# adamjorr/kbbq

Measured on AMD Instinct MI355X. Metric: recalibrated Gbases/sec, higher is better.
Workload: dtype u64

## Files before the change

### kbbq_amd/csrc/bucket.h

```cpp
#pragma once
#include <hip/hip_runtime.h>
#include <stdint.h>

#include "device_common.h"

namespace kbbq {

constexpr int SUB_BITS = 12;
constexpr int NB2_BITS = 9;
constexpr int SUB_BLOCKS = 1 << SUB_BITS;
constexpr int NB2 = 1 << NB2_BITS;
constexpr int L1_SHIFT = SUB_BITS + NB2_BITS;
constexpr int MAX_NB1 = 512;
constexpr int N_XCD = 8;
constexpr int CNT_STRIDE = 32;
constexpr int BK_THREADS = 512;
constexpr int EMIT_GRID = 512;

struct BucketDev {
    unsigned long long *l1;
    uint32_t *l1_cnt;
    uint32_t *l2;
    uint32_t *l2_cnt;
    uint32_t *tickets;
    unsigned long long *direct;
    uint32_t cap1, cap2;
    int nb1;
    int n_src;
    int cnt_stride;
    uint32_t n_sub;
};

__device__ __forceinline__ int xcc_id() {
    unsigned x;
    asm volatile("s_getreg_b32 %0, hwreg(HW_REG_XCC_ID, 0, 4)" : "=s"(x));
    return (int)(x & (N_XCD - 1));
}

__device__ __forceinline__ uint32_t block_scan512(uint32_t v, uint32_t *wave_tot, uint32_t *total) {
    const int lane = threadIdx.x & 63, w = threadIdx.x >> 6;
    uint32_t inc = v;
#pragma unroll
    for (int o = 1; o < 64; o <<= 1) { const uint32_t y = __shfl_up(inc, o); if (lane >= o) inc += y; }
    if (lane == 63) wave_tot[w] = inc;
    __syncthreads();
    uint32_t before = 0, all = 0;
#pragma unroll
    for (int i = 0; i < 8; ++i) { const uint32_t t = wave_tot[i]; before += i < w ? t : 0; all += t; }
    *total = all;
    return before + inc - v;
}

template <int NW, int CH, bool BY_BASE, int RPW, bool PRIV, bool DENSE = true>
__global__ void __launch_bounds__(BK_THREADS) k_emit_marked(ReadsDev R, KParams K, FiltDev F, BucketDev B, const uint64_t *mask,
                                                             uint64_t mask_words, const uint64_t *kofs,
                                                             unsigned long long *inserted) {
    using S = Stage<NW>;
    constexpr int SLOTS = RPW * CH;
    extern __shared__ unsigned long long sorted[];
    __shared__ uint32_t stage[8][DENSE ? RPW : 1][2 * S::WORDS];
    __shared__ uint32_t hist[MAX_NB1], ofs_l[MAX_NB1], gbase_l[MAX_NB1], fill_l[MAX_NB1], wave_tot[8];
    const int lane = threadIdx.x & 63;
    const int w = __builtin_amdgcn_readfirstlane(threadIdx.x >> 6);
    uint32_t *L32 = stage[w][0];
    const int k = K.k;
    const int src = PRIV ? (int)blockIdx.x : xcc_id();
    const uint64_t reads_per_tile = 8 * RPW;
    const uint64_t n_tiles = (R.n_reads + reads_per_tile - 1) / reads_per_tile;
    unsigned long long mine = 0, direct = 0;
    hist[threadIdx.x] = 0;
    if (PRIV) fill_l[threadIdx.x] = (int)threadIdx.x < B.nb1 ? B.l1_cnt[(size_t)src * B.nb1 + threadIdx.x] : 0u;
    __syncthreads();
    uint64_t off[RPW], kb[RPW], word[RPW];
    uint32_t len[RPW];
    auto fetch_tile = [&](uint64_t tile) {
        const uint64_t r0 = (tile * 8 + w) * RPW;
#pragma unroll
        for (int rr = 0; rr < RPW; ++rr) {
            off[rr] = 0; kb[rr] = 0; word[rr] = 0; len[rr] = 0;
            if (r0 + rr < R.n_reads) {
                read_span(R, r0 + rr, off[rr], len[rr]);
                kb[rr] = BY_BASE ? off[rr] : kmer_base(kofs, r0 + rr, R.read_len, k);
                word[rr] = stage_fetch<NW>(R, nullptr, mask, kb[rr], mask_words - 1, off[rr], lane);
            }
        }
    };
    if (blockIdx.x < n_tiles) fetch_tile(blockIdx.x);
    for (uint64_t tile = blockIdx.x; tile < n_tiles; tile += gridDim.x) {
        unsigned long long rec[SLOTS];
        int rk[SLOTS];
#pragma unroll
        for (int s = 0; s < SLOTS; ++s) { rec[s] = 0; rk[s] = -1; }
        if (DENSE) {
            unsigned long long *wlist = sorted + (size_t)w * SLOTS * 64;
            int n_dense = 0;
            __builtin_amdgcn_wave_barrier();
            if (lane < S::WORDS) {
#pragma unroll
                for (int rr = 0; rr < RPW; ++rr) stage_store(stage[w][rr], lane, word[rr]);
            }
            __builtin_amdgcn_wave_barrier();
#pragma unroll
            for (int rr = 0; rr < RPW; ++rr) {
                const int nk = (int)len[rr] - k + 1;
                if (nk > 0) {
                    const uint32_t *L32 = stage[w][rr];
                    const int o31 = (int)(off[rr] & 31), o63 = (int)(off[rr] & 63), x63 = (int)(kb[rr] & 63);
#pragma unroll
                    for (int c = 0; c < CH; ++c) {
                        if (c * 64 < nk) {
                            const int s = c * 64 + lane;
                            const bool marked = lds_bit(L32 + 2 * S::X, x63 + s) != 0;
                            const bool valid = (lds_window32(L32 + 2 * S::M, o63 + s) & K.nmask_bits) == 0;
                            const bool take = s < nk && marked && (BY_BASE || valid);
                            const unsigned long long bal = __ballot(take);
                            if (take) wlist[n_dense + __popcll(bal & ((1ULL << lane) - 1))] = lds_window64(L32 + 2 * S::B, 2 * (o31 + s));
                            n_dense += (int)__popcll(bal);
                            if (!BY_BASE && R.hint_sampled) or_bits64(R.hint_sampled, off[rr] + (uint64_t)c * 64, bal, lane);
                            mine += __popcll(bal);
                        }
                    }
                }
            }
            __builtin_amdgcn_wave_barrier();
#pragma unroll
            for (int i = 0; i < SLOTS; ++i) {
                if (i * 64 < n_dense && i * 64 + lane < n_dense) {
                    const uint64_t key = canon_key(wlist[i * 64 + lane], K);
                    const uint32_t blk = block_of(F, key);
                    rec[i] = ((unsigned long long)blk << 16) | pattern_of(F, key);
                    rk[i] = (int)atomicAdd(&hist[blk >> L1_SHIFT], 1u);
                }
            }
        } else {
#pragma unroll
        for (int rr = 0; rr < RPW; ++rr) {
            const int nk = (int)len[rr] - k + 1;
            if (nk > 0) {
                __builtin_amdgcn_wave_barrier();
                if (lane < S::WORDS) stage_store(L32, lane, word[rr]);
                __builtin_amdgcn_wave_barrier();
                const int o31 = (int)(off[rr] & 31), o63 = (int)(off[rr] & 63), x63 = (int)(kb[rr] & 63);
#pragma unroll
                for (int c = 0; c < CH; ++c) {
                    if (c * 64 < nk) {
                        const int s = c * 64 + lane;
                        const bool marked = lds_bit(L32 + 2 * S::X, x63 + s) != 0;
                        const bool valid = (lds_window32(L32 + 2 * S::M, o63 + s) & K.nmask_bits) == 0;
                        const bool take = s < nk && marked && (BY_BASE || valid);
                        const uint64_t key = canon_key(lds_window64(L32 + 2 * S::B, 2 * (o31 + s)), K);
                        const uint32_t blk = block_of(F, key);
                        rec[rr * CH + c] = ((unsigned long long)blk << 16) | pattern_of(F, key);
                        if (take) rk[rr * CH + c] = (int)atomicAdd(&hist[blk >> L1_SHIFT], 1u);
                        const unsigned long long bal = __ballot(take);
                        if (!BY_BASE && R.hint_sampled) or_bits64(R.hint_sampled, off[rr] + (uint64_t)c * 64, bal, lane);
                        mine += __popcll(bal);
                    }
                }
            }
        }
        }
        if (tile + gridDim.x < n_tiles) fetch_tile(tile + gridDim.x);
        __syncthreads();
        const uint32_t cnt = hist[threadIdx.x];
        hist[threadIdx.x] = 0;
        uint32_t g = 0;
        if (PRIV) {
            g = fill_l[threadIdx.x];
            fill_l[threadIdx.x] = g + cnt;
        } else if (cnt) {
            g = atomicAdd(&B.l1_cnt[((size_t)src * B.nb1 + threadIdx.x) * CNT_STRIDE], cnt);
        }
        uint32_t total;
        const uint32_t ex = block_scan512(cnt, wave_tot, &total);
        ofs_l[threadIdx.x] = ex;
        gbase_l[threadIdx.x] = g;
        __syncthreads();
#pragma unroll
        for (int s = 0; s < SLOTS; ++s)
            if (rk[s] >= 0) sorted[ofs_l[(uint32_t)(rec[s] >> (16 + L1_SHIFT))] + (uint32_t)rk[s]] = rec[s];
        __syncthreads();
        for (uint32_t i = threadIdx.x; i < total; i += BK_THREADS) {
            const unsigned long long v = sorted[i];
            const uint32_t b = (uint32_t)(v >> (16 + L1_SHIFT));
            const uint32_t pos = gbase_l[b] + (i - ofs_l[b]);
            if (pos < B.cap1) {
                B.l1[((size_t)src * B.nb1 + b) * B.cap1 + pos] = v;
            } else {
                bloom_put(F, (uint32_t)(v >> 16), (uint32_t)(v & 0xFFFFu));
                ++direct;
            }
        }
        if (DENSE) __syncthreads();
    }
    if (PRIV && (int)threadIdx.x < B.nb1) B.l1_cnt[(size_t)src * B.nb1 + threadIdx.x] = fill_l[threadIdx.x];
    if (inserted && lane == 0 && mine) atomicAdd(inserted, mine);
    if (direct) atomicAdd(B.direct, direct);
}

constexpr int SPLIT_PER_THREAD = 12;
constexpr int SPLIT_TILE = BK_THREADS * SPLIT_PER_THREAD;

__global__ void __launch_bounds__(BK_THREADS) k_split(FiltDev F, BucketDev B, uint32_t chunks_per_region) {
    __shared__ uint32_t hist[NB2], ofs_l[NB2], gbase_l[NB2], wave_tot[8], unit_l;
    __shared__ uint32_t sorted[SPLIT_TILE];
    __shared__ uint16_t sorted_b[SPLIT_TILE];
    const int home = xcc_id();
    unsigned long long direct = 0;
    hist[threadIdx.x] = 0;
    for (int qi = 0; qi < N_XCD; ++qi) {
        const int q = (home + qi) & (N_XCD - 1);
        const uint32_t n_buckets = B.nb1 > q ? (uint32_t)(B.nb1 - q + N_XCD - 1) / N_XCD : 0;
        const uint32_t n_units = n_buckets * (uint32_t)B.n_src * chunks_per_region;
        for (;;) {
            __syncthreads();
            if (threadIdx.x == 0) unit_l = atomicAdd(&B.tickets[q * CNT_STRIDE], 1u);
            __syncthreads();
            const uint32_t unit = unit_l;
            if (unit >= n_units) break;
            const uint32_t chunk = unit % chunks_per_region, rest = unit / chunks_per_region;
            const int x = (int)(rest % (uint32_t)B.n_src), b1 = q + (int)(rest / (uint32_t)B.n_src) * N_XCD;
            const size_t region = (size_t)x * B.nb1 + b1;
            const uint32_t n = min(B.l1_cnt[region * B.cnt_stride], B.cap1);
            const uint32_t first = chunk * (uint32_t)SPLIT_TILE;
            if (first >= n) continue;
            const uint32_t m = min((uint32_t)SPLIT_TILE, n - first);
            const unsigned long long *src = B.l1 + region * B.cap1 + first;
            uint32_t rec[SPLIT_PER_THREAD];
            int rk[SPLIT_PER_THREAD];
#pragma unroll
            for (int j = 0; j < SPLIT_PER_THREAD; ++j) {
                const uint32_t i = j * BK_THREADS + threadIdx.x;
                rk[j] = -1;
                rec[j] = 0;
                if (i < m) {
                    const unsigned long long v = src[i];
                    rec[j] = (uint32_t)v;
                    rk[j] = (int)atomicAdd(&hist[(uint32_t)(v >> (16 + SUB_BITS)) & (NB2 - 1)], 1u);
                    rk[j] |= (int)(((uint32_t)(v >> (16 + SUB_BITS)) & (NB2 - 1)) << 16);
                }
            }
            __syncthreads();
            const uint32_t cnt = hist[threadIdx.x];
            hist[threadIdx.x] = 0;
            uint32_t g = 0;
            if (cnt) g = atomicAdd(&B.l2_cnt[(size_t)b1 * NB2 + threadIdx.x], cnt);
            uint32_t total;
            const uint32_t ex = block_scan512(cnt, wave_tot, &total);
            ofs_l[threadIdx.x] = ex;
            gbase_l[threadIdx.x] = g;
            __syncthreads();
#pragma unroll
            for (int j = 0; j < SPLIT_PER_THREAD; ++j)
                if (rk[j] >= 0) {
                    const uint32_t b2 = (uint32_t)rk[j] >> 16, at = ofs_l[b2] + ((uint32_t)rk[j] & 0xFFFFu);
                    sorted[at] = rec[j] & 0x0FFFFFFFu;
                    sorted_b[at] = (uint16_t)b2;
                }
            __syncthreads();
            for (uint32_t i = threadIdx.x; i < total; i += BK_THREADS) {
                const uint32_t v = sorted[i], b2 = sorted_b[i];
                const uint32_t pos = gbase_l[b2] + (i - ofs_l[b2]);
                const size_t sub = (size_t)b1 * NB2 + b2;
                if (pos < B.cap2) {
                    B.l2[sub * B.cap2 + pos] = v;
                } else {
                    bloom_put(F, (uint32_t)(sub << SUB_BITS) | (v >> 16), v & 0xFFFFu);
                    ++direct;
                }
            }
        }
    }
    if (direct) atomicAdd(B.direct, direct);
}

constexpr int APPLY_THREADS = 1024;

__global__ void __launch_bounds__(APPLY_THREADS) k_apply(FiltDev F, BucketDev B) {
// ... 46 lines not shown
```

### kbbq_amd/csrc/engine.hip

```cpp
#include <hip/hip_runtime.h>

#include <algorithm>
#include <climits>
#include <cstdarg>
#include <cstdio>
#include <cstdlib>
#include <cstring>
#include <map>
#include <mutex>
#include <string>
#include <thread>
#include <vector>

#include "../../include/kbbq_engine.h"
#include "abi_internal.h"
#include "correct.h"
#include "correct_wave.h"
#include "device_common.h"
#include "host_model.h"

using namespace kbbq;

static thread_local char g_err[512] = "";
int kbbq_fail(int code, const char *fmt, ...) {
    va_list ap;
    va_start(ap, fmt);
    vsnprintf(g_err, sizeof g_err, fmt, ap);
    va_end(ap);
    return code;
}
#define fail kbbq_fail
#define HIP_TRY(expr)                                                                                  \
    do {                                                                                               \
        hipError_t _e = (expr);                                                                        \
        if (_e != hipSuccess)                                                                          \
            return fail(_e == hipErrorOutOfMemory ? KBBQ_ENOMEM : KBBQ_EIO, "%s: %s (%s:%d)", #expr,   \
                        hipGetErrorString(_e), __FILE__, __LINE__);                                    \
    } while (0)

#include "kernels.h"
#include "bucket.h"
#include "long_reads.h"
#include "fixed_compare.h"


struct FilterHost {
    FilterSpec spec;
    uint64_t *d_table = nullptr;
    uint64_t *d_patterns = nullptr;
    unsigned long long *d_inserted = nullptr;
    uint64_t table_bytes() const { return spec.n_blocks * kEngineBlockBytes; }
    FiltDev dev() const {
        FiltDev f;
        f.table = reinterpret_cast<ulonglong2 *>(d_table);
        f.patterns = reinterpret_cast<const ulonglong2 *>(d_patterns);
        f.n_blocks = spec.n_blocks;
        const ModMagic mm = make_mod_magic(spec.n_blocks);
        f.mod_magic = mm.m64;
        f.mod_m32 = mm.m32;
        f.salt0 = spec.salt[0];
        f.salt1 = spec.salt[1];
        return f;
    }
};

struct ProfileSlot {
    std::string name;
    uint64_t launches = 0;
    double ms = 0;
};
struct PendingEvent {
    int slot;
    hipEvent_t a, b;
};

constexpr int kNoOverride = INT_MIN;
struct Options {
    bool no_overlap = false;
    bool no_fastpath = false;
    bool lane_walk = false;
    bool no_pass4_pipeline = false;
    int pass2_side = 2;
    bool tally_general = false;
    bool infer_subset = true;
    bool debug_bucket = false;
    int bucket = -1;
    uint64_t bucket_records = 0;
    uint64_t pass4_piece = 0;
    int scan_blocks = -1;
    int walk_blocks = -1;
    int infer_blocks = 0;
    int subset_edge = kNoOverride;
    int subset_pmask = kNoOverride;
};


enum Scratch {
    S_KMER_PREFIX,
    S_HOST_OUT,
    S_HOST_FLAGS,
    S_DRAW0, S_DRAW1,
    S_TAKE1,
    S_READ_INDEX0, S_READ_INDEX1,
    S_TMASK, S_DIRTY, S_LIST, S_ERR, S_PATCH,
    S_OFFCASE_LIST,
    S_WALK_WORDS,
    S_SIDE1,
    S_COUNT = S_SIDE1 + (S_SIDE1 - S_TMASK),
    S_TAKE0 = S_ERR + (S_SIDE1 - S_TMASK),
};
constexpr int per_side(Scratch name, int side) { return name + side * (S_SIDE1 - S_TMASK); }

struct SideCounters { unsigned long long list_len, queries; };
struct Counters {
    SideCounters side0;
    unsigned long long kmer_total;
    unsigned long long infer_fetched;
    SideCounters side1;
    unsigned long long offcase_len[2];
    SideCounters *side(int s) { return s ? &side1 : &side0; }
};
struct Tickets {
    unsigned int infer, scan[2], walk[2], unused[11];
};
struct Totals {
    unsigned long long walk_reads, walk_queries;
    unsigned long long digest, unused;
};
static_assert(sizeof(Counters) == 64 && offsetof(Counters, kmer_total) == 16 && offsetof(Counters, side1) == 32 && offsetof(Counters, offcase_len) == 48, "d_counters");
static_assert(sizeof(Tickets) == 64 && offsetof(Tickets, scan) == 4 && offsetof(Tickets, walk) == 12, "d_tickets");
static_assert(sizeof(Totals) == 32 && offsetof(Totals, digest) == 16, "d_totals");

struct Pass3 {
    int side;
    hipStream_t stream;
    int stream_no;
    unsigned long long *cnt;
    unsigned int *scan_ticket, *wave_ticket;
    bool shared;
};

struct kbbq_engine {
    kbbq_params p;
    Options opt;
    KParams K;
    hipStream_t stream = nullptr;
    hipStream_t stream2 = nullptr;
    hipEvent_t ev_main = nullptr, ev_side[2] = {nullptr, nullptr};
    hipEvent_t ev_draw = nullptr, ev_ins[2] = {nullptr, nullptr};
    bool ins_pending[2] = {false, false};
    int draw_turn = 0;
    bool side_busy[2] = {false, false};
    Totals *d_totals = nullptr;
    int side_turn = 0;
    uint32_t *d_qpresent = nullptr;
    uint32_t qpresent[8] = {};
    bool qpresent_known = false;
    uint8_t *d_dq_qslot = nullptr;
    int dq_slots = 0;
    uint32_t *d_rg_present[2] = {nullptr, nullptr};
    FilterHost filt[2];
    Xoshiro256 seed_state;
    uint64_t draw_threshold = 0;
    bool draw_always = false;
    bool thresholds_set = false;
    std::vector<int32_t> thresholds;
    unsigned long long *d_hist = nullptr;
// ... 520 lines not shown
        if (!b.est_pending && b.h_inserted) {
            HIP_TRY(hipMemcpyAsync(b.h_inserted, e->filt[1].d_inserted, 8, hipMemcpyDeviceToHost, e->stream));
            HIP_TRY(hipEventRecord(b.ev_est, e->stream));
            b.est_pending = true;
            b.est_bases = b.bases_since[1] + b.cur_bases;
            b.est_prev = b.inserted_at_flush[1];
            if (!b.est_known) {
                HIP_TRY(hipEventSynchronize(b.ev_est));
                bucket_poll_estimate(e);
                b.est_known = true;
            }
        }
    }
    if (e->opt.debug_bucket) fprintf(stderr, "[bucket] flush %d of filter %d: estimate %.3g records over %llu bases (%.4f per base), barrier %d\n",
                       (int)b.flushes[w], w, b.pending_est[w], (unsigned long long)b.bases_since[w], w ? b.frac_trusted : 0.0, (int)barrier);
    b.bases_since[w] = 0;
    b.pending[w] = false;
    b.pending_est[w] = 0;
    b.flushes[w] += 1;
    return KBBQ_OK;
}

int bucket_flush_all(kbbq_engine *e) {
    for (int w = 0; w < 2; ++w) {
        int rc = bucket_flush(e, w);
        if (rc) return rc;
    }
    return KBBQ_OK;
}

int settle(kbbq_engine *e) {
    int rc = bucket_flush_all(e);
    return rc ? rc : sync_engine(e);
}

int bucket_reserve(kbbq_engine *e, int w, double est, uint64_t bases) {
    kbbq_engine::Buckets &b = e->bk;
    int rc = bucket_flush(e, 1 - w);
    if (rc) return rc;
    b.cur_bases = bases;
    if (b.pending[w] && b.pending_est[w] + est > 0.93 * (double)b.capacity) {
        if ((rc = bucket_flush(e, w, false))) return rc;
        if (w == 1) est = (est - 4096.0) / std::max(1e-9, b.frac_used) * b.frac_trusted + 4096.0;
    }
    b.cur_bases = 0;
    b.pending[w] = true;
    b.pending_est[w] += est;
    b.bases_since[w] += bases;
    return KBBQ_OK;
}

}


extern "C" {

const char *kbbq_last_error(void) { return g_err; }

int kbbq_engine_create(const kbbq_params *params, kbbq_engine **out) {
    if (!params || !out) return fail(KBBQ_EINVAL, "null argument");
    if (params->k < 1 || params->k > KBBQ_MAX_KMER) return fail(KBBQ_ERANGE, "k must be <= %d and > 0", KBBQ_MAX_KMER);
    if (params->n_rg < 1 || params->n_rg > 65535) return fail(KBBQ_EINVAL, "n_rg must be in 1..65535");
    if (params->max_read_len < 1 || params->max_read_len > KBBQ_MAX_READ_LEN)
        return fail(KBBQ_ERANGE, "max_read_len must be in 1..%d", KBBQ_MAX_READ_LEN);
    int ndev = 0;
    if (hipGetDeviceCount(&ndev) != hipSuccess || ndev == 0) return fail(KBBQ_ENODEV, "no HIP device visible");
    if (params->device < 0 || params->device >= ndev) return fail(KBBQ_ENODEV, "device %d of %d", params->device, ndev);
    DeviceGuard create_guard(params->device);
    HIP_TRY(create_guard.err);
    kbbq_engine *e = new kbbq_engine;
    e->p = *params;
    {
        Options &o = e->opt;
        auto env_set = [](const char *name) { const char *v = getenv(name); return v && *v; };
        auto env_int = [](const char *name, int dflt) { const char *v = getenv(name); return v && *v ? atoi(v) : dflt; };
        const int fl = params->flags;
        o.no_overlap = (fl & KBBQ_F_NO_OVERLAP) || env_set("KBBQ_NO_OVERLAP");
        o.no_fastpath = (fl & KBBQ_F_NO_FASTPATH) || env_set("KBBQ_NO_FASTPATH");
        o.lane_walk = (fl & KBBQ_F_LANE_WALK) || (getenv("KBBQ_CORRECT") && !strcmp(getenv("KBBQ_CORRECT"), "lane"));
        o.no_pass4_pipeline = (fl & KBBQ_F_NO_PASS4_PIPELINE) || env_set("KBBQ_NO_PASS4_PIPELINE");
        o.pass2_side = (fl & KBBQ_F_PASS2_INORDER) ? 0 : env_int("KBBQ_PASS2_SIDE", o.pass2_side);
        o.tally_general = env_set("KBBQ_TALLY_GENERAL");
        o.infer_subset = env_int("KBBQ_INFER_SUBSET", 1) != 0;
        o.debug_bucket = env_set("KBBQ_DEBUG_BUCKET");
        o.bucket = (fl & KBBQ_F_BUCKET_ON) ? 1 : (fl & KBBQ_F_BUCKET_OFF) ? 0 : env_set("KBBQ_BUCKET") ? (env_int("KBBQ_BUCKET", 0) != 0 ? 1 : 0) : -1;
        o.bucket_records = env_u64("KBBQ_BUCKET_RECORDS", 0);
        o.pass4_piece = env_u64("KBBQ_PASS4_PIECE", 0);
        o.scan_blocks = env_int("KBBQ_SCAN_BLOCKS", o.scan_blocks);
        o.walk_blocks = env_int("KBBQ_WALK_BLOCKS", o.walk_blocks);
        o.infer_blocks = env_int("KBBQ_INFER_BLOCKS", o.infer_blocks);
        o.subset_edge = env_int("KBBQ_SUBSET_EDGE", o.subset_edge);
        o.subset_pmask = env_int("KBBQ_SUBSET_PMASK", o.subset_pmask);
    }
    e->K.k = params->k;
    e->K.shift = 2u * (unsigned)(params->k - 1);
    e->K.mask = params->k < 32 ? ((1ULL << (2 * params->k)) - 1) : ~0ULL;
    e->K.nmask_bits = params->k < 32 ? ((1u << params->k) - 1) : 0xFFFFFFFFu;
    const double fprs[2] = {params->fpr_sampled, params->fpr_trusted};
    for (int w = 0; w < 2; ++w) {
        if (!make_filter_spec(params->approx_kmers, fprs[w], params->bloom_seed, e->filt[w].spec)) {
            delete e;
            return fail(KBBQ_EINVAL, "Error: Invalid bloom filter parameters. Adjust parameters and try again.");
        }
    }
    hipError_t he = hipStreamCreateWithFlags(&e->stream, hipStreamNonBlocking);
    if (he == hipSuccess) he = hipStreamCreateWithFlags(&e->stream2, hipStreamNonBlocking);
    if (he == hipSuccess) he = hipStreamCreateWithFlags(&e->copy, hipStreamNonBlocking);
    for (hipEvent_t *ev : engine_events(e))
        if (he == hipSuccess) he = hipEventCreateWithFlags(ev, hipEventDisableTiming);
    if (he == hipSuccess) he = hipHostMalloc((void **)&e->bk.h_inserted, 64, hipHostMallocDefault);
    if (he != hipSuccess) { kbbq_engine_destroy(e); return fail(KBBQ_EIO, "hipStreamCreate: %s", hipGetErrorString(he)); }
#define CREATE_TRY(expr)                                                                           \
    do {                                                                                           \
        hipError_t _e = (expr);                                                                    \
        if (_e != hipSuccess) {                                                                    \
            int code = _e == hipErrorOutOfMemory ? KBBQ_ENOMEM : KBBQ_EIO;                         \
            fail(code, "%s: %s", #expr, hipGetErrorString(_e));                                    \
            kbbq_engine_destroy(e);                                                                \
            return code;                                                                           \
        }                                                                                          \
    } while (0)
    CREATE_TRY(hipMalloc(&e->d_counters, sizeof(Counters)));
    CREATE_TRY(hipMemset(e->d_counters, 0, sizeof(Counters)));
    CREATE_TRY(hipMalloc(&e->d_tickets, sizeof(Tickets)));
    CREATE_TRY(hipMemset(e->d_tickets, 0, sizeof(Tickets)));
    CREATE_TRY(hipMalloc(&e->d_totals, sizeof(Totals)));
    CREATE_TRY(hipMemset(e->d_totals, 0, sizeof(Totals)));
    CREATE_TRY(hipMalloc(&e->d_dq_qslot, KBBQ_NQ));
    CREATE_TRY(hipMalloc(&e->d_qpresent, 32));
    for (int i = 0; i < 2; ++i) CREATE_TRY(hipMalloc(&e->d_rg_present[i], (((size_t)params->n_rg + 31) / 32) * 4 + 4));
    for (int w = 0; w < 2; ++w) {
        FilterHost &f = e->filt[w];
        CREATE_TRY(hipMalloc(&f.d_table, f.table_bytes()));
        CREATE_TRY(hipMalloc(&f.d_patterns, kNumPatterns * kEngineBlockBytes));
        CREATE_TRY(hipMalloc(&f.d_inserted, 8));
        std::vector<uint64_t> packed(kNumPatterns * 2);
        for (uint64_t i = 0; i < kNumPatterns; ++i) {
            if (!squeeze_block(&f.spec.patterns[i * 8], &packed[i * 2])) {
                kbbq_engine_destroy(e);
                return fail(KBBQ_ESTATE, "pattern %llu uses a bit outside the 128 the generator can reach", (unsigned long long)i);
            }
        }
        CREATE_TRY(hipMemcpy(f.d_patterns, packed.data(), kNumPatterns * kEngineBlockBytes, hipMemcpyHostToDevice));
    }
    e->hist_cycle_words = (uint64_t)params->n_rg * kNQ * 2 * params->max_read_len * 2;
    e->hist_dinuc_words = (uint64_t)params->n_rg * kNQ * 16 * 2;
    CREATE_TRY(hipMalloc(&e->d_hist, (e->hist_cycle_words + e->hist_dinuc_words) * 8));
    CREATE_TRY(hipMalloc(&e->d_dq_base, (size_t)params->n_rg * kNQ * 2));
    CREATE_TRY(hipMalloc(&e->d_dq_cycle, (size_t)params->n_rg * kNQ * 2 * params->max_read_len));
    CREATE_TRY(hipMalloc(&e->d_dq_dinuc, (size_t)params->n_rg * kNQ * 16));
    CREATE_TRY(hipMemcpyToSymbol(HIP_SYMBOL(c_jump), xoshiro_jump_table(), 64 * 4 * 8));
    e->seed_state.seed32(params->seed);
    e->draw_threshold = bernoulli_threshold(params->alpha, &e->draw_always);
    int rc = kbbq_engine_reset(e);
    if (rc) { kbbq_engine_destroy(e); return rc; }
    CREATE_TRY(hipDeviceSynchronize());
    *out = e;
    return KBBQ_OK;
}

void kbbq_engine_destroy(kbbq_engine *e) {
    if (!e) return;
    DeviceGuard destroy_guard(e->p.device);
    if (e->stream) { hipStreamSynchronize(e->stream); }
    if (e->stream2) hipStreamSynchronize(e->stream2);
    if (e->copy) hipStreamSynchronize(e->copy);
// ... 4 lines not shown
    if (e->copy) hipStreamDestroy(e->copy);
    if (e->bk.h_inserted) hipHostFree(e->bk.h_inserted);
    for (int w = 0; w < 2; ++w) {
        hipFree(e->filt[w].d_table);
        hipFree(e->filt[w].d_patterns);
        hipFree(e->filt[w].d_inserted);
    }
    hipFree(e->d_hist);
    hipFree(e->d_dq_base);
    hipFree(e->d_dq_cycle);
    hipFree(e->d_dq_dinuc);
    hipFree(e->d_counters);
    hipFree(e->d_tickets);
    hipFree(e->d_totals);
    hipFree(e->d_dq_qslot);
    hipFree(e->d_qpresent);
    hipFree(e->d_rg_present[0]);
    hipFree(e->d_rg_present[1]);
    hipFree(e->d_qcum);
    hipFree(e->d_errthr);
    hipFree(e->bk.l1); hipFree(e->bk.l2); hipFree(e->bk.l1_cnt); hipFree(e->bk.l2_cnt); hipFree(e->bk.tickets); hipFree(e->bk.direct);
    for (int i = 0; i < S_COUNT; ++i) hipFree(e->scratch[i]);
    if (e->stream2) { hipStreamSynchronize(e->stream2); hipStreamDestroy(e->stream2); }
    if (e->stream) hipStreamDestroy(e->stream);
    delete e;
}

int kbbq_engine_reset(kbbq_engine *e) {
    ENGINE_DEVICE(e);
    int rc0 = sync_engine(e);
    if (rc0) return rc0;
    for (int w = 0; w < 2; ++w) {
        HIP_TRY(hipMemsetAsync(e->filt[w].d_table, 0, e->filt[w].table_bytes(), e->stream));
        HIP_TRY(hipMemsetAsync(e->filt[w].d_inserted, 0, 8, e->stream));
    }
    HIP_TRY(hipMemsetAsync(e->d_hist, 0, (e->hist_cycle_words + e->hist_dinuc_words) * 8, e->stream));
    HIP_TRY(hipMemsetAsync(e->d_counters, 0, sizeof(Counters), e->stream));
    HIP_TRY(hipMemsetAsync(e->d_totals, 0, offsetof(Totals, digest), e->stream));
    HIP_TRY(hipMemsetAsync(e->d_qpresent, 0, 32, e->stream));
    memset(e->qpresent, 0, sizeof e->qpresent);
    e->qpresent_known = false;
    if (e->bk.allocated) {
        HIP_TRY(hipMemsetAsync(e->bk.l1_cnt, 0, kL1CntBytes, e->stream));
        HIP_TRY(hipMemsetAsync(e->bk.l2_cnt, 0, kL2CntBytes, e->stream));
        HIP_TRY(hipMemsetAsync(e->bk.direct, 0, 8, e->stream));
    }
    e->bk.est_pending = false;
    e->bk.est_known = false;
    e->bk.frac_trusted = 0.75;
    e->bk.stream[0] = e->bk.stream[1] = nullptr;
    for (int w = 0; w < 2; ++w) { e->bk.pending[w] = false; e->bk.pending_est[w] = 0; e->bk.bases_since[w] = 0; e->bk.inserted_at_flush[w] = 0; e->bk.flushes[w] = 0; }
    e->thresholds_set = false;
    e->dq_set = false;
    memset(e->stats, 0, sizeof e->stats);
    return sync_engine(e);
}

int kbbq_engine_sync(kbbq_engine *e) {
    ENGINE_DEVICE(e);
    return settle(e);
}

void *kbbq_engine_stream(kbbq_engine *e) { return e ? (void *)e->stream : nullptr; }

int kbbq_engine_dims(kbbq_engine *e, uint64_t *n_rg, uint64_t *n_cycle) {
    if (!e) return fail(KBBQ_EINVAL, "null engine");
    if (n_rg) *n_rg = (uint64_t)e->p.n_rg;
    if (n_cycle) *n_cycle = (uint64_t)e->p.max_read_len;
    return KBBQ_OK;
}

int kbbq_engine_tune(kbbq_engine *e, const char *name, uint64_t value) {
    if (!e || !name) return fail(KBBQ_EINVAL, "null argument");
    if (!strcmp(name, "bucket_records")) {
        if (e->bk.allocated) return fail(KBBQ_ESTATE, "the record buffers are allocated already");
        e->opt.bucket_records = value;
    } else if (!strcmp(name, "pass4_piece")) {
        e->opt.pass4_piece = value;
    } else if (!strcmp(name, "scan_blocks") || !strcmp(name, "walk_blocks") || !strcmp(name, "infer_blocks")) {
        if (value > 17) return fail(KBBQ_EINVAL, "%s: 0 (as many as fit) to 16 workgroups per CU, 17 = default", name);
        (name[0] == 's' ? e->opt.scan_blocks : name[0] == 'w' ? e->opt.walk_blocks : e->opt.infer_blocks) = value == 17 ? (name[0] == 'i' ? 0 : -1) : (int)value;
    } else if (!strcmp(name, "infer_subset")) {
        e->opt.infer_subset = value != 0;
    } else if (!strcmp(name, "pass2_side") || !strcmp(name, "no_overlap")) {
        ENGINE_DEVICE(e);
        int rc = settle(e);
        if (rc) return rc;
        if (name[0] == 'p' && value > 2) return fail(KBBQ_EINVAL, "pass2_side: 0, 1 or 2");
        if (name[0] == 'p') e->opt.pass2_side = (int)value; else e->opt.no_overlap = value != 0;
        e->bk.stream[0] = e->bk.stream[1] = nullptr;
    } else {
        return fail(KBBQ_EINVAL, "unknown knob '%s'", name);
    }
    return KBBQ_OK;
}

int kbbq_filter_info_get(kbbq_engine *e, int which, kbbq_filter_info *out) {
    ENGINE_DEVICE(e);
    if (!out || which < 0 || which > 1) return fail(KBBQ_EINVAL, "bad argument");
    int rc = settle(e);
    if (rc) return rc;
    const FilterSpec &s = e->filt[which].spec;
    memset(out, 0, sizeof *out);
    out->bits = s.bits;
    out->bits_unblocked = s.bits_unblocked;
    out->n_blocks = s.n_blocks;
    out->table_bytes = e->filt[which].table_bytes();
    out->random_seed = s.random_seed;
    out->n_hash = s.n_hash;
    out->n_salt = s.n_salt;
    for (uint32_t i = 0; i < s.n_salt; ++i) out->salt[i] = s.salt[i];
    HIP_TRY(hipMemcpy(&out->inserted, e->filt[which].d_inserted, 8, hipMemcpyDeviceToHost));
    return KBBQ_OK;
}

void *kbbq_filter_device_table(kbbq_engine *e, int which) {
    if (!e || which < 0 || which > 1) return nullptr;
    DeviceGuard guard(e->p.device);
    if (guard.err != hipSuccess || bucket_flush_all(e) != KBBQ_OK) return nullptr;
    return e->filt[which].d_table;
}
void *kbbq_filter_device_counter(kbbq_engine *e, int which) { return e && which >= 0 && which < 2 ? e->filt[which].d_inserted : nullptr; }

int kbbq_filter_download(kbbq_engine *e, int which, uint64_t *host_words, uint64_t n_words) {
    ENGINE_DEVICE(e);
    if (!host_words || which < 0 || which > 1) return fail(KBBQ_EINVAL, "bad argument");
    const uint64_t n_blocks = e->filt[which].spec.n_blocks;
    if (n_words != n_blocks * 8) return fail(KBBQ_EINVAL, "filter has %llu words", (unsigned long long)n_blocks * 8);
    int rc = settle(e);
    if (rc) return rc;
    const uint64_t chunk = 1 << 20;
    std::vector<uint64_t> packed(chunk * 2);
    for (uint64_t b0 = 0; b0 < n_blocks; b0 += chunk) {
        const uint64_t nb = std::min(chunk, n_blocks - b0);
        HIP_TRY(hipMemcpy(packed.data(), e->filt[which].d_table + b0 * 2, nb * kEngineBlockBytes, hipMemcpyDeviceToHost));
        for (uint64_t b = 0; b < nb; ++b) expand_block(&packed[b * 2], host_words + (b0 + b) * 8);
    }
    return KBBQ_OK;
}

int kbbq_filter_patterns_download(kbbq_engine *e, int which, uint64_t *host_words) {
    ENGINE_DEVICE(e);
    if (!host_words || which < 0 || which > 1) return fail(KBBQ_EINVAL, "bad argument");
    std::vector<uint64_t> packed(kNumPatterns * 2);
    HIP_TRY(hipMemcpy(packed.data(), e->filt[which].d_patterns, kNumPatterns * kEngineBlockBytes, hipMemcpyDeviceToHost));
    for (uint64_t i = 0; i < kNumPatterns; ++i) expand_block(&packed[i * 2], host_words + i * 8);
    return KBBQ_OK;
}

int kbbq_filter_or_from(kbbq_engine *e, int which, const void *src_device, uint64_t word_offset, uint64_t n_words) {
    ENGINE_DEVICE(e);
    { int frc = bucket_flush_all(e); if (frc) return frc; }
    if (!src_device || which < 0 || which > 1) return fail(KBBQ_EINVAL, "bad argument");
    const uint64_t total = e->filt[which].spec.n_blocks * 2;
    if (word_offset > total || n_words > total - word_offset || (word_offset & 1)) return fail(KBBQ_EINVAL, "range outside the filter");
    if (!n_words) return KBBQ_OK;
    Timed t(e, "k_or_words");
    hipLaunchKernelGGL(k_or_words, dim3((unsigned)((n_words / 2 + 256) / 256)), dim3(256), 0, e->stream,
                       e->filt[which].d_table + word_offset, (const uint64_t *)src_device, n_words);
    HIP_TRY(hipGetLastError());
    return KBBQ_OK;
}

int kbbq_device_or(kbbq_engine *e, void *dst_device, const void *src_device, uint64_t n_words) {
    ENGINE_DEVICE(e);
    if (!dst_device || !src_device) return fail(KBBQ_EINVAL, "bad argument");
// ... 375 lines not shown
}

int kbbq_device_memory(int32_t device, uint64_t *free_bytes, uint64_t *total_bytes) {
    int cur = 0;
    HIP_TRY(hipGetDevice(&cur));
    if (device >= 0 && device != cur) HIP_TRY(hipSetDevice(device));
    size_t f = 0, t = 0;
    HIP_TRY(hipMemGetInfo(&f, &t));
    if (device >= 0 && device != cur) HIP_TRY(hipSetDevice(cur));
    if (free_bytes) *free_bytes = f;
    if (total_bytes) *total_bytes = t;
    return KBBQ_OK;
}

int kbbq_count_kmer_positions(kbbq_engine *e, const kbbq_reads *reads, uint64_t *out) {
    ENGINE_DEVICE(e);
    if (!reads || !out) return fail(KBBQ_EINVAL, "null argument");
    HostBatchDone host_done(e, reads);
    ReadsDev R; int max_len;
    int rc = device_view(e, reads, &R, &max_len, false);
    if (rc) return rc;
    const uint64_t *kofs;
    return kmer_prefix(e, R, &kofs, out);
}

}

constexpr int kStagedMax = 512;
constexpr int kTallyMaxWindows = 24;
template <template <int> class Launcher, typename... Args>
static int dispatch_nw(int max_len, Args... args) {
    if (max_len <= 192) return Launcher<3>::go(args...);
    if (max_len <= 320) return Launcher<5>::go(args...);
    return Launcher<8>::go(args...);
}

template <int NW> struct LaunchSample {
    static int go(kbbq_engine *e, ReadsDev R, const uint64_t *mask, uint64_t mask_words, const uint64_t *kofs) {
        Timed t(e, "k_insert_sampled");
        hipLaunchKernelGGL((k_insert_marked<NW, false>), dim3(wave_grid(R.n_reads)), dim3(256), 0, e->stream, R, e->K,
                           e->filt[0].dev(), mask, mask_words, kofs, e->filt[0].d_inserted);
        HIP_TRY(hipGetLastError());
        return KBBQ_OK;
    }
};

template <int NW, int CH, int RPW>
static int launch_emit(kbbq_engine *e, int w, ReadsDev R, const uint64_t *mask, uint64_t mask_words, const uint64_t *kofs,
                       unsigned long long *inserted) {
    const BucketDev B = bucket_dev(e, w);
    const uint64_t n_tiles = (R.n_reads + 8 * RPW - 1) / (8 * RPW);
    const int grid = (int)std::min<uint64_t>(n_tiles, EMIT_GRID);
    const size_t lds = (size_t)8 * RPW * CH * 64 * 8;
    hipStream_t st = bucket_stream(e, w);
    Timed t(e, w ? "k_emit_trusted" : "k_emit_sampled", st);
#define KBBQ_EMIT(BYB)                                                                                                        \
    do {                                                                                                                      \
        const void *fn = (const void *)k_emit_marked<NW, CH, BYB, RPW, true, true>;                                            \
        size_t &raised = e->attr_lds_correct[fn];                                                                             \
        if (lds > 48 * 1024 && lds > raised) {                                                                                \
            HIP_TRY(hipFuncSetAttribute(fn, hipFuncAttributeMaxDynamicSharedMemorySize, (int)lds));                            \
            raised = lds;                                                                                                     \
        }                                                                                                                     \
        hipLaunchKernelGGL((k_emit_marked<NW, CH, BYB, RPW, true, true>), dim3(grid), dim3(BK_THREADS), lds, st, R, e->K,      \
                           e->filt[w].dev(), B, mask, mask_words, kofs, inserted);                                            \
    } while (0)
    if (w == 0) KBBQ_EMIT(false); else KBBQ_EMIT(true);
#undef KBBQ_EMIT
    HIP_TRY(hipGetLastError());
    return KBBQ_OK;
}

static int dispatch_emit(kbbq_engine *e, int w, int max_len, ReadsDev R, const uint64_t *mask, uint64_t mask_words, const uint64_t *kofs,
                         unsigned long long *inserted) {
    const int max_nk = std::max(1, max_len - e->p.k + 1);
    if (max_len <= 192) {
        if (max_nk <= 128) return launch_emit<3, 2, 4>(e, w, R, mask, mask_words, kofs, inserted);
        return launch_emit<3, 3, 4>(e, w, R, mask, mask_words, kofs, inserted);
    }
    if (max_len <= 320) return launch_emit<5, 5, 2>(e, w, R, mask, mask_words, kofs, inserted);
    return launch_emit<8, 8, 1>(e, w, R, mask, mask_words, kofs, inserted);
}

extern "C" {

int kbbq_sample_batch(kbbq_engine *e, const kbbq_reads *reads, uint64_t first_kmer_ordinal) {
    ENGINE_DEVICE(e);
    HostBatchDone host_done(e, reads);
    ReadsDev R; int max_len;
    int rc = device_view(e, reads, &R, &max_len, false);
    if (rc) return rc;
    const uint64_t *kofs; uint64_t n_draws;
    if ((rc = kmer_prefix(e, R, &kofs, &n_draws))) return rc;
    if (n_draws == 0) return KBBQ_OK;
    const bool overlap = reads->on_device && !e->opt.no_overlap;
    const int turn = overlap ? e->draw_turn : 0;
    uint64_t *mask;
    if ((rc = scratch_buf(e, turn ? S_DRAW1 : S_DRAW0, (n_draws / 64 + 2) * 8, &mask))) return rc;
    hipStream_t ds = overlap ? e->stream2 : e->stream;
    if (overlap) {
        e->draw_turn ^= 1;
        if (e->ins_pending[turn]) HIP_TRY(hipStreamWaitEvent(ds, e->ev_ins[turn], 0));
    }
    {
        Timed t(e, "k_draw_mask", ds);
        const uint64_t lanes = (n_draws + DRAWS_PER_LANE - 1) / DRAWS_PER_LANE;
        uint64_t st[4];
        xoshiro_state_at(e->p.seed, first_kmer_ordinal, st);
        hipLaunchKernelGGL(k_draw_mask, dim3((unsigned)((lanes + 255) / 256)), dim3(256), 0, ds,
                           st[0], st[1], st[2], st[3],
                           (uint64_t)0, n_draws, e->draw_threshold, e->draw_always ? 1 : 0, mask);
        HIP_TRY(hipGetLastError());
    }
    if (overlap && (rc = run_after(e->stream, ds, e->ev_draw))) return rc;
    if (max_len > kStagedMax) {
        Timed t(e, "k_insert_sampled_long");
        hipLaunchKernelGGL(k_insert_marked_long<false>, dim3(wave_grid(R.n_reads)), dim3(256), 0, e->stream, R, e->K, e->filt[0].dev(),
                           (const uint64_t *)mask, n_draws / 64 + 2, kofs, e->filt[0].d_inserted);
        HIP_TRY(hipGetLastError());
        rc = KBBQ_OK;
    } else if (bucket_on(e, 0)) {
        if ((rc = bucket_reserve(e, 0, (double)n_draws * std::min(1.0, e->p.alpha) * 1.01 + 4096.0, R.n_bases))) return rc;
        rc = dispatch_emit(e, 0, max_len, R, (const uint64_t *)mask, n_draws / 64 + 2, kofs, e->filt[0].d_inserted);
    } else {
        rc = dispatch_nw<LaunchSample>(max_len, e, R, (const uint64_t *)mask, n_draws / 64 + 2, kofs);
    }
    if (!rc) {
        HIP_TRY(hipEventRecord(e->ev_ins[turn], e->stream));
        e->ins_pending[turn] = true;
    }
    return rc;
}

int kbbq_sample_finish(kbbq_engine *e, uint64_t *inserted) {
    ENGINE_DEVICE(e);
    int rc = settle(e);
    if (rc) return rc;
    if (inserted) HIP_TRY(hipMemcpy(inserted, e->filt[0].d_inserted, 8, hipMemcpyDeviceToHost));
    return KBBQ_OK;
}

int kbbq_compute_thresholds(kbbq_engine *e, const char *alpha_text, int32_t *thresholds_out, double *fpr_out,
                            char *p_text_out, size_t p_text_len) {
    ENGINE_DEVICE(e);
    if (!alpha_text) return fail(KBBQ_EINVAL, "null argument");
    int rc = settle(e);
    if (rc) return rc;
    uint64_t inserted = 0;
    HIP_TRY(hipMemcpy(&inserted, e->filt[0].d_inserted, 8, hipMemcpyDeviceToHost));
    if (inserted == 0) return fail(KBBQ_ESTATE, "no k-mers were sampled");
    double fpr = 0;
    std::string p_text;
    e->thresholds = thresholds_from_counts(e->p.k, e->filt[0].spec.bits, inserted, e->filt[0].spec.n_salt, alpha_text, &fpr, &p_text);
    if (fpr_out) *fpr_out = fpr;
    if (p_text_out && p_text_len) snprintf(p_text_out, p_text_len, "%s", p_text.c_str());
    if (thresholds_out) memcpy(thresholds_out, e->thresholds.data(), (e->p.k + 1) * 4);
    rc = kbbq_set_thresholds(e, e->thresholds.data(), e->p.k + 1);
    if (rc) return rc;
    return fpr > .15 ? 1 : 0;
}

int kbbq_set_thresholds(kbbq_engine *e, const int32_t *thresholds, int32_t n) {
    ENGINE_DEVICE(e);
    if (!thresholds) return fail(KBBQ_EINVAL, "null argument");
    if (n != e->p.k + 1) return fail(KBBQ_EINVAL, "expected k+1 = %d thresholds", e->p.k + 1);
    if (thresholds != e->thresholds.data()) e->thresholds.assign(thresholds, thresholds + n);
    e->thresholds_set = true;
    return KBBQ_OK;
}

}


static bool infer_subset_plan(const std::vector<int> &thr, int k, int *edge_out, int *pmask_out) {
    if (k < 8 || (int)thr.size() < k + 1) return false;
    for (int period = 4; period <= 16; period *= 2) {
        if ((k + period - 1) / period > k - thr[k] - 1) continue;
        for (int edge = 0; edge < k; ++edge) {
            bool ok = true;
            for (int n = edge + 1; n <= k && ok; ++n)
                ok = (n - edge + period - 1) / period <= n - thr[n] - 1;
            if (ok) { *edge_out = edge; *pmask_out = period - 1; return true; }
        }
    }
    return false;
}

static Thresholds fill_thresholds(const kbbq_engine *e) {
    Thresholds thr;
    memset(&thr, 0, sizeof thr);
    for (size_t i = 0; i < e->thresholds.size() && i <= KBBQ_MAX_KMER; ++i) thr.v[i] = e->thresholds[i];
    return thr;
}

template <int NW> struct LaunchTrusted {
    static int go(kbbq_engine *e, ReadsDev R, uint32_t *take_bits, uint32_t *err_out, int max_len) {
        const Thresholds thr = fill_thresholds(e);
        HIP_TRY(hipMemsetAsync(&e->d_tickets->infer, 0, 4, e->stream));
        {
            Timed t(e, "k_infer");
            int edge = -1, pmask = 3;
            if (e->opt.infer_subset && !infer_subset_plan(e->thresholds, e->p.k, &edge, &pmask)) edge = -1;
            if (edge >= 0 && e->opt.subset_edge != kNoOverride) edge = e->opt.subset_edge;
            if (edge >= 0 && e->opt.subset_pmask != kNoOverride) pmask = e->opt.subset_pmask;
            const bool short_nk = std::max(1, max_len - e->p.k + 1) <= (NW - 1) * 64;
#define KBBQ_LAUNCH_INFER(NK_, SUB_)                                                                                              \
// ... 794 lines not shown
```

Measured before the change: 24.13.

## Add sparse emit kernel that walks only sampled k-mers from draw mask

Adds k_emit_sparse, which compacts the set bits of the draw mask per wave into an LDS list. It then gathers base windows only for sampled k-mer positions, instead of staging whole reads and testing every k-mer. Hint bits are accumulated in LDS and flushed with atomics. The path is used for fixed-length batches when alpha is below a threshold and draws are not always taken, and an option can force it or disable it. The goal is to avoid reading and processing unsampled bases at low sampling rates. The cost is extra rounds of sort-tail synchronization and scattered global window loads.

```diff
diff --git a/kbbq_amd/csrc/bucket.h b/kbbq_amd/csrc/bucket.h
--- a/kbbq_amd/csrc/bucket.h
+++ b/kbbq_amd/csrc/bucket.h
@@ -49,6 +49,41 @@
     for (int i = 0; i < 8; ++i) { const uint32_t t = wave_tot[i]; before += i < w ? t : 0; all += t; }
     *total = all;
     return before + inc - v;
+}
+
+template <int SLOTS, bool PRIV>
+__device__ __forceinline__ void emit_sort_tail(const FiltDev &F, const BucketDev &B, int src, const unsigned long long (&rec)[SLOTS],
+                                               const int (&rk)[SLOTS], unsigned long long *sorted, uint32_t *hist, uint32_t *ofs_l,
+                                               uint32_t *gbase_l, uint32_t *fill_l, uint32_t *wave_tot, unsigned long long &direct) {
+    const uint32_t cnt = hist[threadIdx.x];
+    hist[threadIdx.x] = 0;
+    uint32_t g = 0;
+    if (PRIV) {
+        g = fill_l[threadIdx.x];
+        fill_l[threadIdx.x] = g + cnt;
+    } else if (cnt) {
+        g = atomicAdd(&B.l1_cnt[((size_t)src * B.nb1 + threadIdx.x) * CNT_STRIDE], cnt);
+    }
+    uint32_t total;
+    const uint32_t ex = block_scan512(cnt, wave_tot, &total);
+    ofs_l[threadIdx.x] = ex;
+    gbase_l[threadIdx.x] = g;
+    __syncthreads();
+#pragma unroll
+    for (int s = 0; s < SLOTS; ++s)
+        if (rk[s] >= 0) sorted[ofs_l[(uint32_t)(rec[s] >> (16 + L1_SHIFT))] + (uint32_t)rk[s]] = rec[s];
+    __syncthreads();
+    for (uint32_t i = threadIdx.x; i < total; i += BK_THREADS) {
+        const unsigned long long v = sorted[i];
+        const uint32_t b = (uint32_t)(v >> (16 + L1_SHIFT));
+        const uint32_t pos = gbase_l[b] + (i - ofs_l[b]);
+        if (pos < B.cap1) {
+            B.l1[((size_t)src * B.nb1 + b) * B.cap1 + pos] = v;
+        } else {
+            bloom_put(F, (uint32_t)(v >> 16), (uint32_t)(v & 0xFFFFu));
+            ++direct;
+        }
+    }
 }
 
 template <int NW, int CH, bool BY_BASE, int RPW, bool PRIV, bool DENSE = true>
@@ -162,38 +197,127 @@
         }
         if (tile + gridDim.x < n_tiles) fetch_tile(tile + gridDim.x);
         __syncthreads();
-        const uint32_t cnt = hist[threadIdx.x];
-        hist[threadIdx.x] = 0;
-        uint32_t g = 0;
-        if (PRIV) {
-            g = fill_l[threadIdx.x];
-            fill_l[threadIdx.x] = g + cnt;
-        } else if (cnt) {
-            g = atomicAdd(&B.l1_cnt[((size_t)src * B.nb1 + threadIdx.x) * CNT_STRIDE], cnt);
-        }
-        uint32_t total;
-        const uint32_t ex = block_scan512(cnt, wave_tot, &total);
-        ofs_l[threadIdx.x] = ex;
-        gbase_l[threadIdx.x] = g;
+        emit_sort_tail<SLOTS, PRIV>(F, B, src, rec, rk, sorted, hist, ofs_l, gbase_l, fill_l, wave_tot, direct);
+        if (DENSE) __syncthreads();
+    }
+    if (PRIV && (int)threadIdx.x < B.nb1) B.l1_cnt[(size_t)src * B.nb1 + threadIdx.x] = fill_l[threadIdx.x];
+    if (inserted && lane == 0 && mine) atomicAdd(inserted, mine);
+    if (direct) atomicAdd(B.direct, direct);
+}
+
+constexpr int SP_DRAWS = 64 * 16;
+constexpr int SP_SLOTS = 5;
+constexpr int SP_HINT_WORDS = 160;
+
+__global__ void __launch_bounds__(BK_THREADS) k_emit_sparse(ReadsDev R, KParams K, FiltDev F, BucketDev B, const uint16_t *mask16,
+                                                             uint64_t n_draws, unsigned long long *inserted) {
+    extern __shared__ unsigned long long sorted[];
+    __shared__ uint16_t list[8][SP_DRAWS];
+    __shared__ uint32_t hint_l[8][SP_HINT_WORDS];
+    __shared__ uint32_t hist[MAX_NB1], ofs_l[MAX_NB1], gbase_l[MAX_NB1], fill_l[MAX_NB1], wave_tot[8], span_marks[2][8];
+    const int lane = threadIdx.x & 63;
+    const int w = __builtin_amdgcn_readfirstlane(threadIdx.x >> 6);
+    const int src = (int)blockIdx.x;
+    const uint32_t nk = R.read_len - (uint32_t)K.k + 1;
+    const uint32_t nk_magic = nk > 1 ? (uint32_t)((0x100000000ULL + nk - 1) / nk) : 0u;
+    const uint32_t hint_words = ((nk + SP_DRAWS - 2) / nk * R.read_len + nk + 31) / 32 + 2;
+    const bool hint_lds = hint_words <= SP_HINT_WORDS;
+    const uint64_t n_spans = (n_draws + SP_DRAWS - 1) / SP_DRAWS;
+    const uint64_t n_tiles = (n_spans + 7) / 8;
+    unsigned long long mine = 0, direct = 0;
+    hist[threadIdx.x] = 0;
+    fill_l[threadIdx.x] = (int)threadIdx.x < B.nb1 ? B.l1_cnt[(size_t)src * B.nb1 + threadIdx.x] : 0u;
+    for (int i = lane; i < SP_HINT_WORDS; i += 64) hint_l[w][i] = 0;
+    __syncthreads();
+    uint16_t *my = list[w];
+    auto fetch_bits = [&](uint64_t tile) -> uint32_t {
+        const uint64_t g = (tile * 8 + w) * 64 + lane, first = g * 16;
+        uint32_t v = 0;
+        if (first < n_draws) {
+            v = mask16[g];
+            if (n_draws - first < 16) v &= (1u << (uint32_t)(n_draws - first)) - 1;
+        }
+        return v;
+    };
+    uint32_t next_bits = blockIdx.x < n_tiles ? fetch_bits(blockIdx.x) : 0u;
+    int par = 0;
+    for (uint64_t tile = blockIdx.x; tile < n_tiles; tile += gridDim.x, par ^= 1) {
+        uint32_t bits = next_bits;
+        const uint32_t c = __popc(bits);
+        uint32_t inc = c;
+#pragma unroll
+        for (int o = 1; o < 64; o <<= 1) { const uint32_t y = __shfl_up(inc, o); if (lane >= o) inc += y; }
+        const uint32_t n_marks = (uint32_t)__builtin_amdgcn_readlane((int)inc, 63);
+        for (uint32_t at = inc - c; bits; bits &= bits - 1) my[at++] = (uint16_t)(lane * 16 + __ffs(bits) - 1);
+        if (lane == 0) span_marks[par][w] = n_marks;
+        if (tile + gridDim.x < n_tiles) next_bits = fetch_bits(tile + gridDim.x);
+        const uint64_t j0 = (tile * 8 + w) * SP_DRAWS;
+        uint64_t r0; uint32_t s0;
+        if ((j0 >> 32) == 0) { r0 = (uint32_t)j0 / nk; s0 = (uint32_t)j0 % nk; }
+        else { r0 = j0 / nk; s0 = (uint32_t)(j0 % nk); }
+        const uint64_t b0 = r0 * R.read_len;
+        const uint32_t b32 = (uint32_t)(b0 & 31), hw0 = (b32 + s0) >> 5;
         __syncthreads();
-#pragma unroll
-        for (int s = 0; s < SLOTS; ++s)
-            if (rk[s] >= 0) sorted[ofs_l[(uint32_t)(rec[s] >> (16 + L1_SHIFT))] + (uint32_t)rk[s]] = rec[s];
-        __syncthreads();
-        for (uint32_t i = threadIdx.x; i < total; i += BK_THREADS) {
-            const unsigned long long v = sorted[i];
-            const uint32_t b = (uint32_t)(v >> (16 + L1_SHIFT));
-            const uint32_t pos = gbase_l[b] + (i - ofs_l[b]);
-            if (pos < B.cap1) {
-                B.l1[((size_t)src * B.nb1 + b) * B.cap1 + pos] = v;
-            } else {
-                bloom_put(F, (uint32_t)(v >> 16), (uint32_t)(v & 0xFFFFu));
-                ++direct;
-            }
-        }
-        if (DENSE) __syncthreads();
-    }
-    if (PRIV && (int)threadIdx.x < B.nb1) B.l1_cnt[(size_t)src * B.nb1 + threadIdx.x] = fill_l[threadIdx.x];
+        uint32_t most = 0;
+#pragma unroll
+        for (int i = 0; i < 8; ++i) most = max(most, span_marks[par][i]);
+        const uint32_t n_rounds = (most + SP_SLOTS * 64 - 1) / (SP_SLOTS * 64);
+        for (uint32_t rd = 0; rd < n_rounds; ++rd) {
+            unsigned long long rec[SP_SLOTS];
+            int rk[SP_SLOTS];
+            uint64_t win[SP_SLOTS];
+            uint32_t nm[SP_SLOTS], rel[SP_SLOTS];
+#pragma unroll
+            for (int i = 0; i < SP_SLOTS; ++i) {
+                rec[i] = 0; rk[i] = -1; win[i] = 0; nm[i] = 0; rel[i] = 0;
+                const uint32_t m = (rd * SP_SLOTS + i) * 64 + lane;
+                if (m < n_marks) {
+                    const uint32_t t = s0 + my[m];
+                    const uint32_t q = nk > 1 ? __umulhi(t, nk_magic) : t;
+                    rel[i] = q * R.read_len + (t - q * nk);
+                    const uint64_t b = b0 + rel[i];
+                    win[i] = window64(R.bases, 2 * b);
+                    nm[i] = (uint32_t)window64(R.nmask, b);
+                }
+            }
+#pragma unroll
+            for (int i = 0; i < SP_SLOTS; ++i) {
+                const uint32_t m0 = (rd * SP_SLOTS + i) * 64;
+                if (m0 < n_marks) {
+                    const bool live = m0 + lane < n_marks;
+                    const bool valid = live && (nm[i] & K.nmask_bits) == 0;
+                    mine += __popcll(__ballot(valid));
+                    if (valid && R.hint_sampled) {
+                        if (hint_lds) {
+                            const uint32_t x = b32 + rel[i];
+                            atomicOr(&hint_l[w][(x >> 5) - hw0], 1u << (x & 31));
+                        } else {
+                            const uint64_t b = b0 + rel[i];
+                            atomicOr(&R.hint_sampled[b >> 5], 1u << (uint32_t)(b & 31));
+                        }
+                    }
+                    if (valid) {
+                        const uint64_t key = canon_key(win[i], K);
+                        const uint32_t blk = block_of(F, key);
+                        rec[i] = ((unsigned long long)blk << 16) | pattern_of(F, key);
+                        rk[i] = (int)atomicAdd(&hist[blk >> L1_SHIFT], 1u);
+                    }
+                }
+            }
+            __syncthreads();
+            emit_sort_tail<SP_SLOTS, true>(F, B, src, rec, rk, sorted, hist, ofs_l, gbase_l, fill_l, wave_tot, direct);
+        }
+        if (R.hint_sampled && hint_lds && n_marks) {
+            for (uint32_t i = lane; i < hint_words; i += 64) {
+                const uint32_t v = hint_l[w][i];
+                if (v) {
+                    atomicOr(&R.hint_sampled[(b0 >> 5) + hw0 + i], v);
+                    hint_l[w][i] = 0;
+                }
+            }
+        }
+    }
+    if ((int)threadIdx.x < B.nb1) B.l1_cnt[(size_t)src * B.nb1 + threadIdx.x] = fill_l[threadIdx.x];
     if (inserted && lane == 0 && mine) atomicAdd(inserted, mine);
     if (direct) atomicAdd(B.direct, direct);
 }
diff --git a/kbbq_amd/csrc/engine.hip b/kbbq_amd/csrc/engine.hip
--- a/kbbq_amd/csrc/engine.hip
+++ b/kbbq_amd/csrc/engine.hip
@@ -83,6 +83,7 @@
     int pass2_side = 2;
     bool tally_general = false;
     bool infer_subset = true;
+    int emit_sparse = 2;
     bool debug_bucket = false;
     int bucket = -1;
     uint64_t bucket_records = 0;
@@ -769,6 +770,7 @@
         o.pass2_side = (fl & KBBQ_F_PASS2_INORDER) ? 0 : env_int("KBBQ_PASS2_SIDE", o.pass2_side);
         o.tally_general = env_set("KBBQ_TALLY_GENERAL");
         o.infer_subset = env_int("KBBQ_INFER_SUBSET", 1) != 0;
+        o.emit_sparse = std::min(2, std::max(0, env_int("KBBQ_EMIT_SPARSE", o.emit_sparse)));
         o.debug_bucket = env_set("KBBQ_DEBUG_BUCKET");
         o.bucket = (fl & KBBQ_F_BUCKET_ON) ? 1 : (fl & KBBQ_F_BUCKET_OFF) ? 0 : env_set("KBBQ_BUCKET") ? (env_int("KBBQ_BUCKET", 0) != 0 ? 1 : 0) : -1;
         o.bucket_records = env_u64("KBBQ_BUCKET_RECORDS", 0);
@@ -939,6 +941,9 @@
         (name[0] == 's' ? e->opt.scan_blocks : name[0] == 'w' ? e->opt.walk_blocks : e->opt.infer_blocks) = value == 17 ? (name[0] == 'i' ? 0 : -1) : (int)value;
     } else if (!strcmp(name, "infer_subset")) {
         e->opt.infer_subset = value != 0;
+    } else if (!strcmp(name, "emit_sparse")) {
+        if (value > 2) return fail(KBBQ_EINVAL, "emit_sparse: 0 (never), 1 (whenever the batch allows) or 2 (where it wins)");
+        e->opt.emit_sparse = (int)value;
     } else if (!strcmp(name, "pass2_side") || !strcmp(name, "no_overlap")) {
         ENGINE_DEVICE(e);
         int rc = settle(e);
@@ -1480,6 +1485,21 @@
     return launch_emit<8, 8, 1>(e, w, R, mask, mask_words, kofs, inserted);
 }
 
+static int launch_emit_sparse(kbbq_engine *e, ReadsDev R, const uint64_t *mask, uint64_t n_draws, unsigned long long *inserted) {
+    const BucketDev B = bucket_dev(e, 0);
+    const uint64_t n_spans = (n_draws + SP_DRAWS - 1) / SP_DRAWS, n_tiles = (n_spans + 7) / 8;
+    const int grid = (int)std::min<uint64_t>(n_tiles, EMIT_GRID);
+    const size_t lds = (size_t)8 * SP_SLOTS * 64 * 8;
+    hipStream_t st = bucket_stream(e, 0);
+    Timed t(e, "k_emit_sampled", st);
+    hipLaunchKernelGGL(k_emit_sparse, dim3(grid), dim3(BK_THREADS), lds, st, R, e->K, e->filt[0].dev(), B, (const uint16_t *)mask, n_draws,
+                       inserted);
+    HIP_TRY(hipGetLastError());
+    return KBBQ_OK;
+}
+
+constexpr double kEmitSparseAlpha = 0.55;
+
 extern "C" {
 
 int kbbq_sample_batch(kbbq_engine *e, const kbbq_reads *reads, uint64_t first_kmer_ordinal) {
@@ -1519,7 +1539,10 @@
         rc = KBBQ_OK;
     } else if (bucket_on(e, 0)) {
         if ((rc = bucket_reserve(e, 0, (double)n_draws * std::min(1.0, e->p.alpha) * 1.01 + 4096.0, R.n_bases))) return rc;
-        rc = dispatch_emit(e, 0, max_len, R, (const uint64_t *)mask, n_draws / 64 + 2, kofs, e->filt[0].d_inserted);
+        const bool sparse_fits = !R.offsets && !kofs;
+        const bool sparse = sparse_fits && (e->opt.emit_sparse == 1 || (e->opt.emit_sparse == 2 && !e->draw_always && e->p.alpha < kEmitSparseAlpha));
+        rc = sparse ? launch_emit_sparse(e, R, (const uint64_t *)mask, n_draws, e->filt[0].d_inserted)
+                    : dispatch_emit(e, 0, max_len, R, (const uint64_t *)mask, n_draws / 64 + 2, kofs, e->filt[0].d_inserted);
     } else {
         rc = dispatch_nw<LaunchSample>(max_len, e, R, (const uint64_t *)mask, n_draws / 64 + 2, kofs);
     }
```

After: 23.67. 0.981x the previous value.
